# dluvizon/deephar

Measured on NVIDIA H100. Metric: frames/sec (256x256, 16-frame clips, b32), higher is better.
Workload: dtype bf16x3 split (fp32 accumulate, wgmma)

## Files before the change

deephar_b200/csrc/conv_sep.cu:

```cuda
#include "tc_common.cuh"

namespace tcs {
using namespace tc;
using R = tc::Roles<2, 1>;
constexpr int WARP_EPI0 = R::WARP_EPI0, WARP_TMA = R::WARP_TMA, WARP_PATCH = R::WARP_PATCH, NTHREADS = R::NTHREADS,
              REGS_PROD = R::REGS_PROD, REGS_EPI = R::REGS_EPI, REGS_CTRL = R::REGS_CTRL;

constexpr int A_BYTES = BM * 64;
constexpr int NWG = 128;
constexpr int NPW = 1;
constexpr int NA = 4;
constexpr int NB = 3;
constexpr int NP = 3;

struct SepParams {
    TcParams t;
    int patch_stride;
    int patch_bytes;
    int ry, fn;
    int dbg;
};

template <int KS, int TW, bool SHARE, bool BNPRO, bool LO>
__global__ void __launch_bounds__(NTHREADS, 1)
sep_tma_kernel(const __grid_constant__ SepParams SP, const __grid_constant__ CUtensorMap map_hi,
               const __grid_constant__ CUtensorMap map_lo, const __grid_constant__ CUtensorMap map_x) {
    constexpr int PAD = KS / 2;
    constexpr int PC = TW + 2 * PAD;
    constexpr int NR = 4 + KS - 1;
#ifdef DH_ABLATE
    const int DBG = SP.dbg;
#else
    constexpr int DBG = 0;
#endif
    const TcParams& P = SP.t;
    extern __shared__ __align__(1024) uint8_t smem_raw[];
    if (smem_u32(smem_raw) & 1023u) __trap();
    uint8_t* smem = smem_raw;
    const int tid = threadIdx.x;
    const int warp = tid >> 5, lane = tid & 31;
    constexpr bool want_lo = LO;
    const int b_bytes = P.bn_cta * 64;
    uint8_t* b_ring = smem + NA * 2 * A_BYTES;
    uint8_t* patch0 = b_ring + NB * 2 * b_bytes;
    uint64_t* bars = reinterpret_cast<uint64_t*>(patch0 + NP * SP.patch_stride);
    constexpr int NB_A = NA + 2 * NA;
    const uint32_t bar_full0 = smem_u32(bars), bar_empty0 = smem_u32(bars + NA), bar_fullb0 = smem_u32(bars + NB_A),
                   bar_emptyb0 = smem_u32(bars + NB_A + NB), bar_pfull0 = smem_u32(bars + NB_A + 2 * NB),
                   bar_pempty0 = smem_u32(bars + NB_A + 2 * NB + NP);
    const int n0 = blockIdx.y * P.bn_cta;
    const int nkb = P.n_kblocks;
    const uint32_t my_rank = SHARE ? cluster_ctarank() : 0u;

    if (warp == WARP_TMA && lane == 0) {
        tma_prefetch_desc(&map_hi);
        if (want_lo) tma_prefetch_desc(&map_lo);
        tma_prefetch_desc(&map_x);
        for (int s = 0; s < NA; ++s) {
            mbar_init(bar_full0 + 8 * s, SHARE ? 1u : (uint32_t)NWG);
            mbar_init(bar_empty0 + 16 * s, (SHARE ? 2u : 1u) * R::EPQ);
            mbar_init(bar_empty0 + 16 * s + 8, (SHARE ? 2u : 1u) * R::EPQ);
        }
        for (int s = 0; s < NB; ++s) {
            mbar_init(bar_fullb0 + 8 * s, 1);
            mbar_init(bar_emptyb0 + 8 * s, R::EPQ);
        }
        for (int s = 0; s < NP; ++s) {
            mbar_init(bar_pfull0 + 8 * s, 1);
            mbar_init(bar_pempty0 + 8 * s, NWG);
        }
        fence_barrier_init();
    }
    if (SHARE) cluster_sync_all(); else __syncthreads();

    const int tiles_mine = ((int)P.n_mtiles - (int)blockIdx.x + (int)gridDim.x - 1) / (int)gridDim.x;
    const int total_g = tiles_mine * nkb;
    const int n_own = SHARE ? (total_g - (int)my_rank + 1) / 2 : total_g;

    if (warp < WARP_EPI0) {
        reg_prod<REGS_PROD, R::LAUNCH_REGS>();
        const ConvParams& c = P.c;
        const int w = warp >> 2;
        const int tw = tid & (NWG - 1);
        const int cp = tw & 15;
        const int blk = tw >> 4;
        constexpr int XB = TW / 4;
        const int strip = blk / XB, xb = blk - strip * XB;
        const int fn = (strip * 4) / SP.ry, ry = (strip * 4) - fn * SP.ry;
        const int prr = SP.ry + 2 * PAD;
        const float* pbase0 = reinterpret_cast<const float*>(patch0) +
                             ((size_t)((fn * prr + ry) * PC + xb * 4)) * SBK + cp * 2;
        const int row0 = strip * 4 * TW + xb * 4;
        const float lowb = c.pre_relu ? 0.f : -3.402823466e38f;
        unsigned colmask = 0;
        if (BNPRO) {
#pragma unroll
            for (int q = 0; q < NR; ++q) {
                const int ix = xb * 4 + q - PAD;
                if (ix >= 0 && ix < TW) colmask |= 1u << q;
            }
        }
        float2 wt[KS][KS];
        auto load_taps = [&](int jn) {
            const int gn = SHARE ? 2 * jn + (int)my_rank : jn;
            const int kbn = gn % nkb;
            const float* wp = c.w_dw + kbn * SBK + cp * 2;
#pragma unroll
            for (int a = 0; a < KS; ++a)
#pragma unroll
                for (int b = 0; b < KS; ++b)
                    wt[a][b] = __ldg(reinterpret_cast<const float2*>(wp + (size_t)(a * KS + b) * c.Cin));
        };
        if (w < n_own) load_taps(w);
        for (int j = w; j < n_own; j += NPW) {
            const int pb_i = j % NP;
            const uint32_t pfull = bar_pfull0 + 8 * pb_i, pempty = bar_pempty0 + 8 * pb_i;
            const float* pbase = pbase0 + (size_t)pb_i * (SP.patch_stride / 4);
            const int g = SHARE ? 2 * j + (int)my_rank : j;
            const int ti = g / nkb, kb = g - ti * nkb;
            const int ch = kb * SBK + cp * 2;
            float2 acc[4][4];
#pragma unroll
            for (int o = 0; o < 4; ++o)
#pragma unroll
                for (int q = 0; q < 4; ++q) acc[o][q] = make_float2(0.f, 0.f);
            float2 ps = make_float2(1.f, 1.f), pb = make_float2(0.f, 0.f);
            unsigned rowmask = 0;
            if (BNPRO) {
                ps = __ldg(reinterpret_cast<const float2*>(c.pre_scale + ch));
                pb = __ldg(reinterpret_cast<const float2*>(c.pre_shift + ch));
                const int t = blockIdx.x + ti * gridDim.x;
                const int y0 = SP.fn > 1 ? 0 : ((t * BM) / TW) % c.H;
#pragma unroll
                for (int r = 0; r < NR; ++r) {
                    const int iy = y0 + ry + r - PAD;
                    if (iy >= 0 && iy < c.H) rowmask |= 1u << r;
                }
            }

            if (!(DBG & 2)) mbar_wait_relaxed(pfull, (uint32_t)((j / NP) & 1), (DBG & 2048) ? 32u : 0u);
            auto load_row = [&](int r, float2* in) {
#pragma unroll
                for (int q = 0; q < NR; ++q) {
                    float2 v = *reinterpret_cast<const float2*>(pbase + (r * PC + q) * SBK);
                    if (BNPRO) v = ffma2(v, ps, pb);
                    v = make_float2(fmaxf(v.x, lowb), fmaxf(v.y, lowb));
                    if (BNPRO && !(((rowmask >> r) & 1u) && ((colmask >> q) & 1u))) v = make_float2(0.f, 0.f);
                    in[q] = v;
                }
            };
            if (!(DBG & 1)) {
                float2 inb[2][NR];
                load_row(0, inb[0]);
#pragma unroll
                for (int r = 0; r < NR; ++r) {
                    if (r + 1 < NR) load_row(r + 1, inb[(r + 1) & 1]);
                    const float2* in = inb[r & 1];
#pragma unroll
                    for (int kx = 0; kx < KS; ++kx)
#pragma unroll
                        for (int o = 0; o < 4; ++o) {
                            const int ky = r - o;
                            if (ky >= 0 && ky < KS) {
#pragma unroll
                                for (int q = 0; q < 4; ++q) acc[o][q] = ffma2(wt[ky][kx], in[q + kx], acc[o][q]);
                            }
                        }
                }
            }
            if (j + NPW < n_own) load_taps(j + NPW);
            if (!(DBG & 2)) mbar_arrive(pempty);

            const int s = g % NA;
            const uint32_t it = (uint32_t)(g / NA);
            wait_stage_free(bar_empty0, s, it, (DBG & 2048) ? 32u : 0u);
            uint8_t* a_hi = smem + (size_t)s * (2 * A_BYTES);
            uint8_t* a_lo = a_hi + A_BYTES;
#pragma unroll
            for (int o = 0; o < 4; ++o)
#pragma unroll
                for (int q = 0; q < 4; ++q) {
                    uint32_t hi, lo;
                    split2(acc[o][q].x, acc[o][q].y, hi, lo);
                    const uint32_t off = swz64(row0 + o * TW + q, cp * 2);
                    *reinterpret_cast<uint32_t*>(a_hi + off) = hi;
                    if (want_lo) *reinterpret_cast<uint32_t*>(a_lo + off) = lo;
                }
            fence_proxy_async();
            if (SHARE) {
                asm volatile("bar.sync %0, %1;" ::"r"(1 + w), "r"(NWG) : "memory");
                if (tw == 0) {
                    mbar_arrive(bar_full0 + 8 * s);
                    const uint32_t peer = my_rank ^ 1u;
                    const uint32_t peer_full = mapa_peer(bar_full0 + 8 * s, peer);
                    if (!(DBG & 8)) {
                        bulk_s2peer(mapa_peer(smem_u32(a_hi), peer), smem_u32(a_hi), A_BYTES, peer_full);
                        if (want_lo) bulk_s2peer(mapa_peer(smem_u32(a_lo), peer), smem_u32(a_lo), A_BYTES, peer_full);
                    }
                }
            } else {
                mbar_arrive(bar_full0 + 8 * s);
            }
        }
    } else if (warp < WARP_TMA) {
        reg_inc<REGS_EPI>();
        const int wg = (warp - WARP_EPI0) >> 2, wt = tid - 32 * WARP_EPI0 - 128 * wg;
        float acc[R::MH][ACC_N];
        const uint64_t dbase = make_desc64(smem_u32(smem) + (uint32_t)(wg * 64 * 64));
        const uint64_t dbase_b = make_desc64(smem_u32(b_ring));
        const uint32_t sta16 = (2 * A_BYTES) >> 4, stb16 = (uint32_t)(2 * b_bytes) >> 4, alo16 = A_BYTES >> 4,
                       blo16 = (uint32_t)b_bytes >> 4;
        for (int ti = 0; ti < tiles_mine; ++ti) {
            const int g0 = ti * nkb;
            wg_tile<R::MH, SBK / 16, LO>(
                P.bn_cta, acc, nkb, 0u, alo16, blo16, !(DBG & 64),
                [&](int kb, uint64_t& da, uint64_t& db) {
                    const int g = g0 + kb, s = g % NA, sb = g % NB;
                    if (!(DBG & 128)) mbar_wait(bar_full0 + 8 * s, (uint32_t)(g / NA) & 1);
                    mbar_wait(bar_fullb0 + 8 * sb, (uint32_t)(g / NB) & 1);
                    da = dbase + (uint64_t)((uint32_t)s * sta16);
                    db = dbase_b + (uint64_t)((uint32_t)sb * stb16);
                },
                [&](int kb) {
                    const int g = g0 + kb, s = g % NA;
                    wg_release<SHARE>(bar_empty0 + 16 * s + 8 * ((g / NA) & 1), wg, wt, my_rank ^ 1u);
                    if (wt == 0) mbar_arrive(bar_emptyb0 + 8 * (g % NB));
                });
            wg_epilogue<R::MH>(P, acc, ((int)blockIdx.x + ti * (int)gridDim.x) * BM + 64 * wg, n0, wt);
        }
    } else {
        reg_dec<REGS_CTRL>();
        if (warp == WARP_TMA) {
            if (lane == 0) {
                const uint32_t tx = (DBG & 16) ? 0u : (uint32_t)(want_lo ? 2 : 1) * (uint32_t)b_bytes;
                const uint32_t tx_a = (DBG & 8) ? 0u : (uint32_t)(want_lo ? 2 : 1) * (uint32_t)A_BYTES;
                for (int g = 0; g < total_g; ++g) {
                    const int ti = g / nkb, kb = g - ti * nkb;
                    const int sb = g % NB;
                    const uint32_t itb = (uint32_t)(g / NB);
                    if (itb >= 1) mbar_wait_relaxed(bar_emptyb0 + 8 * sb, (itb - 1) & 1, (DBG & 2048) ? 64u : 0u);
                    const uint32_t full = bar_fullb0 + 8 * sb;
                    mbar_arrive_expect_tx(full, tx);
                    const uint32_t b_hi = smem_u32(b_ring + (size_t)sb * (2 * b_bytes));
                    const uint32_t b_lo = b_hi + (uint32_t)b_bytes;
                    if (!(DBG & 16)) {
                        tma_load_2d(b_hi, &map_hi, kb * SBK, n0, full);
                        if (want_lo) tma_load_2d(b_lo, &map_lo, kb * SBK, n0, full);
                    }
                    if (SHARE && (uint32_t)(g & 1) != my_rank) {
                        const int sa = g % NA;
                        wait_stage_free(bar_empty0, sa, (uint32_t)(g / NA));
                        mbar_arrive_expect_tx(bar_full0 + 8 * sa, tx_a);
                    }
                }
            }
        } else if (warp == WARP_PATCH) {
            if (lane == 0 && !(DBG & 2)) {
                const ConvParams& c = P.c;
                auto coords = [&](int j, int& kb, int& nf, int& y0) {
                    const int g = SHARE ? 2 * j + (int)my_rank : j;
                    const int ti = g / nkb;
                    kb = g - ti * nkb;
                    const int t = blockIdx.x + ti * gridDim.x;
                    const int grow = (t * BM) / TW;
                    nf = grow / c.H;
                    y0 = grow - nf * c.H;
                };
                for (int j = 0; j < n_own; ++j) {
                    int kb, nf, y0;
                    coords(j, kb, nf, y0);
                    const int w = j % NP;
                    const int pfd = (DBG & 1024) ? 2 : (DBG & 4096) ? 4 : (DBG & 8192) ? 9 : 0;
                    if (pfd && j + pfd < n_own) {
                        int kb2, nf2, y2;
                        coords(j + pfd, kb2, nf2, y2);
                        tma_prefetch_4d(&map_x, kb2 * SBK, -PAD, y2 - PAD, nf2);
                    }
                    mbar_wait_relaxed(bar_pempty0 + 8 * w, (uint32_t)(((j / NP) & 1) ^ 1), (DBG & 2048) ? 64u : 0u);
                    const uint32_t pf = bar_pfull0 + 8 * w;
                    mbar_arrive_expect_tx(pf, (uint32_t)SP.patch_bytes);
                    tma_load_4d(smem_u32(patch0 + (size_t)w * SP.patch_stride), &map_x, kb * SBK, -PAD, y0 - PAD, nf, pf);
                }
            }
        }
    }
    if (SHARE) cluster_sync_all(); else __syncthreads();
}

static bool make_map_x(CUtensorMap* map, const ConvParams& p, int pc, int prr, int fn) {
    EncodeTiledFn enc = get_encode();
    if (!enc) return false;
    cuuint64_t dims[4] = {(cuuint64_t)p.Cin, (cuuint64_t)p.W, (cuuint64_t)p.H, (cuuint64_t)p.N};
    cuuint64_t strides[3] = {(cuuint64_t)p.ldx * 4, (cuuint64_t)p.W * p.ldx * 4, (cuuint64_t)p.H * p.W * p.ldx * 4};
    cuuint32_t box[4] = {(cuuint32_t)SBK, (cuuint32_t)pc, (cuuint32_t)prr, (cuuint32_t)fn};
    cuuint32_t estr[4] = {1, 1, 1, 1};
    return enc(map, CU_TENSOR_MAP_DATA_TYPE_FLOAT32, 4, const_cast<float*>(p.x), dims, strides, box, estr,
               CU_TENSOR_MAP_INTERLEAVE_NONE, CU_TENSOR_MAP_SWIZZLE_NONE, CU_TENSOR_MAP_L2_PROMOTION_L2_256B,
               CU_TENSOR_MAP_FLOAT_OOB_FILL_NONE) == CUDA_SUCCESS;
}

}

bool dh_sep_tma_supported(const dh_ctx* ctx, const ConvParams& p, const dh_packed_w* packed) {
    if (!ctx->sep_tma) return false;
    if (!packed || !packed->hi || !packed->lo) return false;
    if (!(p.kh == p.kw && (p.kh == 3 || p.kh == 5)) || p.sh != 1 || p.sw != 1) return false;
    if (p.Ho != p.H || p.Wo != p.W) return false;
    if (p.pre_scale && ((reinterpret_cast<uintptr_t>(p.pre_scale) & 7) || (reinterpret_cast<uintptr_t>(p.pre_shift) & 7))) return false;
    if (!(p.W == 32 || p.W == 16 || p.W == 8)) return false;
    const int tr = tc::BM / p.W;
    if (tr <= p.H ? (p.H % tr) != 0 : (tr % p.H) != 0) return false;
    if ((p.Cin % tcs::SBK) != 0 || (p.ldx & 3)) return false;
    if ((reinterpret_cast<uintptr_t>(p.x) & 15) || (reinterpret_cast<uintptr_t>(p.w_dw) & 7)) return false;
    if (packed->cout_pad != dh_tc_cout_pad(p.Cout) || packed->k < p.Cin) return false;
    return true;
}

int dh_launch_sep_tma(dh_ctx* ctx, const ConvParams& p, const dh_packed_w* packed, int precision, cudaStream_t s) {
    using namespace tc;
    using namespace tcs;
    SepParams SP;
    TcParams& P = SP.t;
    P.c = p;
    P.c.K = p.Cin;
    P.k_pad = packed->k;
    P.n_kblocks = p.Cin / SBK;
    int gy;
    tile_n(p.Cout, &P.bn_cta, &gy);
    P.precision = (precision == 1) ? 1 : 3;
    P.ks = p.kh;
    P.n_mtiles = (p.M + BM - 1) / BM;
    P.stages = 2;
    const int pad = p.kh / 2;
    const int tr = BM / p.W;
    SP.ry = tr <= p.H ? tr : p.H;
    SP.fn = tr <= p.H ? 1 : tr / p.H;
    const int pc = p.W + 2 * pad, prr = SP.ry + 2 * pad;
    SP.patch_bytes = SBK * 4 * pc * prr * SP.fn;
    SP.patch_stride = (SP.patch_bytes + 1023) / 1024 * 1024;
#ifdef DH_ABLATE
    SP.dbg = ctx->dbg;
    P.dbg = ctx->dbg;
#else
    SP.dbg = 0;
    P.dbg = 0;
#endif
    const size_t smem = (size_t)NA * 2 * A_BYTES + (size_t)NB * 2 * P.bn_cta * 64 + NP * (size_t)SP.patch_stride + 512;
    if (smem > 227 * 1024) {
        dh_set_error("dh_launch_sep_tma: tile does not fit shared memory");
        return -1;
    }
    CUtensorMap map_hi, map_lo, map_x;
    if (!make_map_b64(&map_hi, packed->hi, packed->k, packed->cout_pad, P.bn_cta) ||
        !make_map_b64(&map_lo, packed->lo, packed->k, packed->cout_pad, P.bn_cta) ||
        !make_map_x(&map_x, p, pc, prr, SP.fn)) {
        dh_set_error("dh_launch_sep_tma: cuTensorMapEncodeTiled failed");
        return -1;
    }
    int gx = ctx->num_sms / gy;
    if (gx < 1) gx = 1;
    if (gx > P.n_mtiles) gx = P.n_mtiles;
    dim3 grid(gx, gy);
    const bool share = gy % 2 == 0 && ctx->share_a;
    cudaError_t e = cudaSuccess;
#define DH_SEP_LAUNCH_(KS_, TW_, BN_, LO_)                                                                              \
    do {                                                                                                         \
        if (share) {                                                                                             \
            e = ensure_smem<sep_tma_kernel<KS_, TW_, true, BN_, LO_>>(smem); \
            if (e == cudaSuccess) {                                                                              \
                cudaLaunchConfig_t cfg = {};                                                                     \
                cfg.gridDim = grid; cfg.blockDim = dim3(NTHREADS); cfg.dynamicSmemBytes = smem; cfg.stream = s;  \
                cudaLaunchAttribute at[1];                                                                       \
                at[0].id = cudaLaunchAttributeClusterDimension;                                                  \
                at[0].val.clusterDim.x = 1; at[0].val.clusterDim.y = 2; at[0].val.clusterDim.z = 1;              \
                cfg.attrs = at; cfg.numAttrs = 1;                                                                \
                e = cudaLaunchKernelEx(&cfg, sep_tma_kernel<KS_, TW_, true, BN_, LO_>, SP, map_hi, map_lo, map_x);    \
            }                                                                                                    \
        } else {                                                                                                 \
            e = ensure_smem<sep_tma_kernel<KS_, TW_, false, BN_, LO_>>(smem); \
            if (e == cudaSuccess) sep_tma_kernel<KS_, TW_, false, BN_, LO_><<<grid, NTHREADS, smem, s>>>(SP, map_hi, map_lo, map_x); \
        }                                                                                                        \
    } while (0)
#define DH_SEP_LAUNCH_P(KS_, TW_, BN_) do { if (P.precision == 3) DH_SEP_LAUNCH_(KS_, TW_, BN_, true); else DH_SEP_LAUNCH_(KS_, TW_, BN_, false); } while (0)
#define DH_SEP_LAUNCH(KS_, TW_) do { if (p.pre_scale) DH_SEP_LAUNCH_P(KS_, TW_, true); else DH_SEP_LAUNCH_P(KS_, TW_, false); } while (0)
    if (p.kh == 5) {
        if (p.W == 32) DH_SEP_LAUNCH(5, 32); else if (p.W == 16) DH_SEP_LAUNCH(5, 16); else DH_SEP_LAUNCH(5, 8);
    } else {
        if (p.W == 32) DH_SEP_LAUNCH(3, 32); else if (p.W == 16) DH_SEP_LAUNCH(3, 16); else DH_SEP_LAUNCH(3, 8);
    }
#undef DH_SEP_LAUNCH
#undef DH_SEP_LAUNCH_P
#undef DH_SEP_LAUNCH_
    if (e != cudaSuccess) {
        dh_set_error("dh_launch_sep_tma: launch setup failed: %s", cudaGetErrorString(e));
        return (int)e;
    }
    return 0;
}
```

deephar_b200/csrc/tc_common.cuh:

```cuda
#pragma once
#include <cuda.h>
#include <cuda_bf16.h>
#include "common.cuh"
#include "conv_params.cuh"

namespace tc {


constexpr int BM = 128;
constexpr int BK = 64;
constexpr int NPROD = 256;
constexpr int MAX_BN_CTA = 96;
constexpr int ACC_N = MAX_BN_CTA / 2;
template <int Q, int NPW = 2>
struct Roles {
    static constexpr int EPQ = Q;
    static constexpr int MH = 2 / Q;
    static constexpr int NEPI = 128 * Q;
    static constexpr int WARP_EPI0 = 4 * NPW;
    static constexpr int WARP_TMA = WARP_EPI0 + 4 * Q, WARP_PATCH = WARP_TMA + 2;
    static constexpr int NTHREADS = 32 * (WARP_TMA + 4);
    static constexpr int REGS_PROD = Q == 1 ? 168 : (NPW == 1 ? 192 : 80), REGS_EPI = 144, REGS_CTRL = 32;
    static constexpr int LAUNCH_REGS = NTHREADS <= 512 ? 128 : 96;
    static_assert(128 * NPW * REGS_PROD + NEPI * REGS_EPI + 128 * REGS_CTRL <= NTHREADS * LAUNCH_REGS,
                  "setmaxnreg budget exceeds the CTA's register allocation: the last setmaxnreg.inc would never return");
};
constexpr int A_TILE_BYTES = BM * 128;
constexpr int MAX_STAGES = 4;

struct TcParams {
    ConvParams c;
    int n_kblocks;
    int bn_cta;
    int stages;
    int precision;
    int ks;
    int k_pad;
    int n_mtiles;
    int dbg;
};

__device__ __forceinline__ uint32_t smem_u32(const void* p) { return (uint32_t)__cvta_generic_to_shared(p); }

__device__ __forceinline__ void mbar_init(uint32_t bar, uint32_t count) {
    asm volatile("mbarrier.init.shared::cta.b64 [%0], %1;" ::"r"(bar), "r"(count));
}
__device__ __forceinline__ void mbar_arrive(uint32_t bar) {
    asm volatile("{\n .reg .b64 st;\n mbarrier.arrive.shared::cta.b64 st, [%0];\n}" ::"r"(bar) : "memory");
}
__device__ __forceinline__ void mbar_arrive_expect_tx(uint32_t bar, uint32_t bytes) {
    asm volatile("{\n .reg .b64 st;\n mbarrier.arrive.expect_tx.shared::cta.b64 st, [%0], %1;\n}" ::"r"(bar), "r"(bytes)
                 : "memory");
}
__device__ __forceinline__ void mbar_wait(uint32_t bar, uint32_t parity) {
    uint32_t ok;
    do {
        asm volatile(
            "{\n .reg .pred p;\n mbarrier.try_wait.parity.shared::cta.b64 p, [%1], %2;\n selp.u32 %0, 1, 0, p;\n}"
            : "=r"(ok)
            : "r"(bar), "r"(parity)
            : "memory");
    } while (!ok);
}
__device__ __forceinline__ void mbar_wait_relaxed(uint32_t bar, uint32_t parity, uint32_t ns) {
    uint32_t ok;
    for (;;) {
        asm volatile(
            "{\n .reg .pred p;\n mbarrier.try_wait.parity.shared::cta.b64 p, [%1], %2;\n selp.u32 %0, 1, 0, p;\n}"
            : "=r"(ok)
            : "r"(bar), "r"(parity)
            : "memory");
        if (ok) break;
        if (ns) __nanosleep(ns);
    }
}
__device__ __forceinline__ void fence_barrier_init() { asm volatile("fence.mbarrier_init.release.cluster;" ::: "memory"); }
__device__ __forceinline__ void fence_proxy_async() { asm volatile("fence.proxy.async.shared::cta;" ::: "memory"); }

__device__ __forceinline__ void tma_load_2d(uint32_t dst, const CUtensorMap* map, int c0, int c1, uint32_t bar) {
    asm volatile(
        "cp.async.bulk.tensor.2d.shared::cluster.global.mbarrier::complete_tx::bytes [%0], [%1, {%2, %3}], [%4];"
        ::"r"(dst), "l"(map), "r"(c0), "r"(c1), "r"(bar)
        : "memory");
}
__device__ __forceinline__ void tma_prefetch_desc(const CUtensorMap* map) {
    asm volatile("prefetch.tensormap [%0];" ::"l"(map) : "memory");
}
__device__ __forceinline__ uint32_t cluster_ctarank() {
    uint32_t r;
    asm volatile("mov.u32 %0, %%cluster_ctarank;" : "=r"(r));
    return r;
}
__device__ __forceinline__ uint32_t mapa_peer(uint32_t local_addr, uint32_t peer) {
    uint32_t r;
    asm volatile("mapa.shared::cluster.u32 %0, %1, %2;" : "=r"(r) : "r"(local_addr), "r"(peer));
    return r;
}
__device__ __forceinline__ void cluster_sync_all() {
    asm volatile("barrier.cluster.arrive.release.aligned;\n\tbarrier.cluster.wait.acquire.aligned;" ::: "memory");
}
__device__ __forceinline__ void bulk_s2peer(uint32_t dst_cluster, uint32_t src_cta, uint32_t bytes, uint32_t bar_cluster) {
    asm volatile("cp.async.bulk.shared::cluster.shared::cta.mbarrier::complete_tx::bytes [%0], [%1], %2, [%3];"
                 ::"r"(dst_cluster), "r"(src_cta), "r"(bytes), "r"(bar_cluster)
                 : "memory");
}
template <int R> __device__ __forceinline__ void reg_inc() { asm volatile("setmaxnreg.inc.sync.aligned.u32 %0;" ::"n"(R)); }
template <int R> __device__ __forceinline__ void reg_dec() { asm volatile("setmaxnreg.dec.sync.aligned.u32 %0;" ::"n"(R)); }
template <int R, int LAUNCH> __device__ __forceinline__ void reg_prod() {
    if constexpr (R > LAUNCH) reg_inc<R>();
    else if constexpr (R < LAUNCH) reg_dec<R>();
}
__device__ __forceinline__ void mbar_arrive_cluster(uint32_t bar_cluster) {
    asm volatile("mbarrier.arrive.release.cluster.shared::cluster.b64 _, [%0];" ::"r"(bar_cluster) : "memory");
}

__device__ __forceinline__ void wgmma_fence() { asm volatile("wgmma.fence.sync.aligned;" ::: "memory"); }
__device__ __forceinline__ void wgmma_commit() { asm volatile("wgmma.commit_group.sync.aligned;" ::: "memory"); }
template <int N> __device__ __forceinline__ void wgmma_wait() { asm volatile("wgmma.wait_group.sync.aligned %0;" ::"n"(N) : "memory"); }
__device__ __forceinline__ void acc_fence(float& r) { asm volatile("" : "+f"(r)::"memory"); }
template <int N> __device__ __forceinline__ void wgmma_bf16(float* d, uint64_t a, uint64_t b, uint32_t acc);
template <> __device__ __forceinline__ void wgmma_bf16<16>(float* d, uint64_t a, uint64_t b, uint32_t acc) {
    asm volatile(
        "{\n .reg .pred p;\n setp.ne.b32 p, %10, 0;\n"
        " wgmma.mma_async.sync.aligned.m64n16k16.f32.bf16.bf16 {%0, %1, %2, %3, %4, %5, %6, %7}, %8, %9, p, 1, 1, 0, 0;\n}"
        : "+f"(d[0]), "+f"(d[1]), "+f"(d[2]), "+f"(d[3]), "+f"(d[4]), "+f"(d[5]), "+f"(d[6]), "+f"(d[7])
        : "l"(a), "l"(b), "r"(acc));
}
template <> __device__ __forceinline__ void wgmma_bf16<32>(float* d, uint64_t a, uint64_t b, uint32_t acc) {
    asm volatile(
        "{\n .reg .pred p;\n setp.ne.b32 p, %18, 0;\n"
        " wgmma.mma_async.sync.aligned.m64n32k16.f32.bf16.bf16 {%0, %1, %2, %3, %4, %5, %6, %7, %8, %9, %10, %11, %12, %13, %14, %15}, %16, %17, p, 1, 1, 0, 0;\n}"
        : "+f"(d[0]), "+f"(d[1]), "+f"(d[2]), "+f"(d[3]), "+f"(d[4]), "+f"(d[5]), "+f"(d[6]), "+f"(d[7]), "+f"(d[8]), "+f"(d[9]), "+f"(d[10]), "+f"(d[11]), "+f"(d[12]), "+f"(d[13]), "+f"(d[14]), "+f"(d[15])
        : "l"(a), "l"(b), "r"(acc));
}
template <> __device__ __forceinline__ void wgmma_bf16<48>(float* d, uint64_t a, uint64_t b, uint32_t acc) {
    asm volatile(
        "{\n .reg .pred p;\n setp.ne.b32 p, %26, 0;\n"
        " wgmma.mma_async.sync.aligned.m64n48k16.f32.bf16.bf16 {%0, %1, %2, %3, %4, %5, %6, %7, %8, %9, %10, %11, %12, %13, %14, %15, %16, %17, %18, %19, %20, %21, %22, %23}, %24, %25, p, 1, 1, 0, 0;\n}"
        : "+f"(d[0]), "+f"(d[1]), "+f"(d[2]), "+f"(d[3]), "+f"(d[4]), "+f"(d[5]), "+f"(d[6]), "+f"(d[7]), "+f"(d[8]), "+f"(d[9]), "+f"(d[10]), "+f"(d[11]), "+f"(d[12]), "+f"(d[13]), "+f"(d[14]), "+f"(d[15]), "+f"(d[16]), "+f"(d[17]), "+f"(d[18]), "+f"(d[19]), "+f"(d[20]), "+f"(d[21]), "+f"(d[22]), "+f"(d[23])
        : "l"(a), "l"(b), "r"(acc));
}
template <> __device__ __forceinline__ void wgmma_bf16<64>(float* d, uint64_t a, uint64_t b, uint32_t acc) {
    asm volatile(
        "{\n .reg .pred p;\n setp.ne.b32 p, %34, 0;\n"
        " wgmma.mma_async.sync.aligned.m64n64k16.f32.bf16.bf16 {%0, %1, %2, %3, %4, %5, %6, %7, %8, %9, %10, %11, %12, %13, %14, %15, %16, %17, %18, %19, %20, %21, %22, %23, %24, %25, %26, %27, %28, %29, %30, %31}, %32, %33, p, 1, 1, 0, 0;\n}"
        : "+f"(d[0]), "+f"(d[1]), "+f"(d[2]), "+f"(d[3]), "+f"(d[4]), "+f"(d[5]), "+f"(d[6]), "+f"(d[7]), "+f"(d[8]), "+f"(d[9]), "+f"(d[10]), "+f"(d[11]), "+f"(d[12]), "+f"(d[13]), "+f"(d[14]), "+f"(d[15]), "+f"(d[16]), "+f"(d[17]), "+f"(d[18]), "+f"(d[19]), "+f"(d[20]), "+f"(d[21]), "+f"(d[22]), "+f"(d[23]), "+f"(d[24]), "+f"(d[25]), "+f"(d[26]), "+f"(d[27]), "+f"(d[28]), "+f"(d[29]), "+f"(d[30]), "+f"(d[31])
        : "l"(a), "l"(b), "r"(acc));
}
template <> __device__ __forceinline__ void wgmma_bf16<80>(float* d, uint64_t a, uint64_t b, uint32_t acc) {
    asm volatile(
        "{\n .reg .pred p;\n setp.ne.b32 p, %42, 0;\n"
        " wgmma.mma_async.sync.aligned.m64n80k16.f32.bf16.bf16 {%0, %1, %2, %3, %4, %5, %6, %7, %8, %9, %10, %11, %12, %13, %14, %15, %16, %17, %18, %19, %20, %21, %22, %23, %24, %25, %26, %27, %28, %29, %30, %31, %32, %33, %34, %35, %36, %37, %38, %39}, %40, %41, p, 1, 1, 0, 0;\n}"
        : "+f"(d[0]), "+f"(d[1]), "+f"(d[2]), "+f"(d[3]), "+f"(d[4]), "+f"(d[5]), "+f"(d[6]), "+f"(d[7]), "+f"(d[8]), "+f"(d[9]), "+f"(d[10]), "+f"(d[11]), "+f"(d[12]), "+f"(d[13]), "+f"(d[14]), "+f"(d[15]), "+f"(d[16]), "+f"(d[17]), "+f"(d[18]), "+f"(d[19]), "+f"(d[20]), "+f"(d[21]), "+f"(d[22]), "+f"(d[23]), "+f"(d[24]), "+f"(d[25]), "+f"(d[26]), "+f"(d[27]), "+f"(d[28]), "+f"(d[29]), "+f"(d[30]), "+f"(d[31]), "+f"(d[32]), "+f"(d[33]), "+f"(d[34]), "+f"(d[35]), "+f"(d[36]), "+f"(d[37]), "+f"(d[38]), "+f"(d[39])
        : "l"(a), "l"(b), "r"(acc));
}
template <> __device__ __forceinline__ void wgmma_bf16<96>(float* d, uint64_t a, uint64_t b, uint32_t acc) {
    asm volatile(
        "{\n .reg .pred p;\n setp.ne.b32 p, %50, 0;\n"
        " wgmma.mma_async.sync.aligned.m64n96k16.f32.bf16.bf16 {%0, %1, %2, %3, %4, %5, %6, %7, %8, %9, %10, %11, %12, %13, %14, %15, %16, %17, %18, %19, %20, %21, %22, %23, %24, %25, %26, %27, %28, %29, %30, %31, %32, %33, %34, %35, %36, %37, %38, %39, %40, %41, %42, %43, %44, %45, %46, %47}, %48, %49, p, 1, 1, 0, 0;\n}"
        : "+f"(d[0]), "+f"(d[1]), "+f"(d[2]), "+f"(d[3]), "+f"(d[4]), "+f"(d[5]), "+f"(d[6]), "+f"(d[7]), "+f"(d[8]), "+f"(d[9]), "+f"(d[10]), "+f"(d[11]), "+f"(d[12]), "+f"(d[13]), "+f"(d[14]), "+f"(d[15]), "+f"(d[16]), "+f"(d[17]), "+f"(d[18]), "+f"(d[19]), "+f"(d[20]), "+f"(d[21]), "+f"(d[22]), "+f"(d[23]), "+f"(d[24]), "+f"(d[25]), "+f"(d[26]), "+f"(d[27]), "+f"(d[28]), "+f"(d[29]), "+f"(d[30]), "+f"(d[31]), "+f"(d[32]), "+f"(d[33]), "+f"(d[34]), "+f"(d[35]), "+f"(d[36]), "+f"(d[37]), "+f"(d[38]), "+f"(d[39]), "+f"(d[40]), "+f"(d[41]), "+f"(d[42]), "+f"(d[43]), "+f"(d[44]), "+f"(d[45]), "+f"(d[46]), "+f"(d[47])
        : "l"(a), "l"(b), "r"(acc));
}

__device__ __forceinline__ uint64_t make_desc(uint32_t smem_addr) {
    return (uint64_t)((smem_addr >> 4) & 0x3FFF) | (1ull << 16) | ((uint64_t)(1024 >> 4) << 32) | (1ull << 62);
}


__device__ __forceinline__ void split2(float a, float b, uint32_t& hi, uint32_t& lo) {
    __nv_bfloat162 h = __floats2bfloat162_rn(a, b);
    float ra = a - __low2float(h), rb = b - __high2float(h);
    __nv_bfloat162 l = __floats2bfloat162_rn(ra, rb);
    hi = *reinterpret_cast<uint32_t*>(&h);
    lo = *reinterpret_cast<uint32_t*>(&l);
}

__device__ __forceinline__ uint32_t swz(int row, int k) {
    return (uint32_t)(row * 128 + ((((k >> 3) ^ (row & 7)) << 4) | ((k & 7) << 1)));
}


constexpr int SBK = 32;
__device__ __forceinline__ void tma_load_4d(uint32_t dst, const CUtensorMap* map, int c0, int c1, int c2, int c3,
                                            uint32_t bar) {
    asm volatile(
        "cp.async.bulk.tensor.4d.shared::cluster.global.mbarrier::complete_tx::bytes [%0], [%1, {%2, %3, %4, %5}], [%6];"
        ::"r"(dst), "l"(map), "r"(c0), "r"(c1), "r"(c2), "r"(c3), "r"(bar)
        : "memory");
}

__device__ __forceinline__ void tma_prefetch_4d(const CUtensorMap* map, int c0, int c1, int c2, int c3) {
    asm volatile("cp.async.bulk.prefetch.tensor.4d.L2.global [%0, {%1, %2, %3, %4}];"
                 ::"l"(map), "r"(c0), "r"(c1), "r"(c2), "r"(c3) : "memory");
}

__device__ __forceinline__ uint64_t make_desc64(uint32_t smem_addr) {
    return (uint64_t)((smem_addr >> 4) & 0x3FFF) | (1ull << 16) | ((uint64_t)(512 >> 4) << 32) | (2ull << 62);
}
__device__ __forceinline__ uint32_t swz64(int row, int k) {
    return (uint32_t)(row * 64 + ((((k >> 3) ^ ((row >> 1) & 3)) << 4) | ((k & 7) << 1)));
}

__device__ __forceinline__ float4 lds128(uint32_t a) {
    float4 v;
    asm volatile("ld.shared.v4.f32 {%0, %1, %2, %3}, [%4];" : "=f"(v.x), "=f"(v.y), "=f"(v.z), "=f"(v.w) : "r"(a) : "memory");
    return v;
}

__device__ __forceinline__ void wait_stage_free(uint32_t bar_empty0, int s, uint32_t it, uint32_t ns = 0) {
    if (it >= 1) mbar_wait_relaxed(bar_empty0 + 16 * s + 8 * ((it - 1) & 1), ((it - 1) >> 1) & 1, ns);
}


template <int N, int MH>
__device__ __forceinline__ void acc_fence_all(float (&acc)[MH][ACC_N]) {
#pragma unroll
    for (int h = 0; h < MH; ++h)
#pragma unroll
        for (int i = 0; i < N / 2; ++i) acc_fence(acc[h][i]);
}

template <int N, int MH, int NK16, bool LO>
__device__ __forceinline__ void wg_issue_kblock(float (&acc)[MH][ACC_N], uint64_t da, uint32_t a_half16, uint32_t alo16,
                                                uint64_t db, uint32_t blo16, bool first) {
    wgmma_fence();
#pragma unroll
    for (int k = 0; k < NK16; ++k) {
        const uint32_t acc0 = (first && k == 0) ? 0u : 1u;
#pragma unroll
        for (int h = 0; h < MH; ++h) {
            const uint64_t a = da + (uint64_t)(h * a_half16 + 2 * k);
            wgmma_bf16<N>(acc[h], a, db + 2 * k, acc0);
            if (LO) {
                wgmma_bf16<N>(acc[h], a + alo16, db + 2 * k, 1u);
                wgmma_bf16<N>(acc[h], a, db + blo16 + 2 * k, 1u);
            }
        }
    }
    wgmma_commit();
}

template <int N, int MH, int NK16, bool LO, class Stage, class Release>
__device__ __forceinline__ void wg_tile_n(float (&acc)[MH][ACC_N], int nkb, uint32_t a_half16, uint32_t alo16,
                                          uint32_t blo16, bool mma, Stage& stage, Release& release) {
    for (int kb = 0; kb < nkb; ++kb) {
        uint64_t da, db;
        stage(kb, da, db);
        if (mma) {
            acc_fence_all<N>(acc);
            wg_issue_kblock<N, MH, NK16, LO>(acc, da, a_half16, alo16, db, blo16, kb == 0);
        }
        wgmma_wait<1>();
        acc_fence_all<N>(acc);
        if (kb > 0) release(kb - 1);
    }
    wgmma_wait<0>();
    acc_fence_all<N>(acc);
    release(nkb - 1);
}

template <int MH, int NK16, bool LO, class Stage, class Release>
__device__ __forceinline__ void wg_tile(int bn, float (&acc)[MH][ACC_N], int nkb, uint32_t a_half16, uint32_t alo16,
                                        uint32_t blo16, bool mma, Stage&& stage, Release&& release) {
    switch (bn) {
    case 16: wg_tile_n<16, MH, NK16, LO>(acc, nkb, a_half16, alo16, blo16, mma, stage, release); break;
    case 32: wg_tile_n<32, MH, NK16, LO>(acc, nkb, a_half16, alo16, blo16, mma, stage, release); break;
    case 48: wg_tile_n<48, MH, NK16, LO>(acc, nkb, a_half16, alo16, blo16, mma, stage, release); break;
    case 64: wg_tile_n<64, MH, NK16, LO>(acc, nkb, a_half16, alo16, blo16, mma, stage, release); break;
    case 80: wg_tile_n<80, MH, NK16, LO>(acc, nkb, a_half16, alo16, blo16, mma, stage, release); break;
    default: wg_tile_n<96, MH, NK16, LO>(acc, nkb, a_half16, alo16, blo16, mma, stage, release); break;
    }
}

template <bool SHARE>
__device__ __forceinline__ void wg_release(uint32_t bar, int wg, int wt, uint32_t peer) {
    asm volatile("bar.sync %0, 128;" ::"r"(4 + wg) : "memory");
    if (wt == 0) {
        mbar_arrive(bar);
        if (SHARE) mbar_arrive_cluster(mapa_peer(bar, peer));
    }
}

__device__ __forceinline__ size_t res1_src(const ConvParams& c, int m) {
    if (!c.up1) return (size_t)m;
    const int hw = c.Ho * c.Wo;
    const int n = m / hw, rem = m - n * hw;
    const int y = rem / c.Wo, x = rem - y * c.Wo;
    return ((size_t)n * (c.Ho >> 1) + (y >> 1)) * (size_t)(c.Wo >> 1) + (size_t)(x >> 1);
}

__device__ __forceinline__ float2 ldg2(const float* p) { return __ldg(reinterpret_cast<const float2*>(p)); }

template <int MH>
__device__ __forceinline__ void wg_epilogue(const TcParams& P, const float (&acc)[MH][ACC_N], int m0, int n0, int wt) {
    const ConvParams& c = P.c;
#ifdef DH_ABLATE
    if (P.dbg & 32) return;
#endif
    const int rq = 16 * (wt >> 5) + ((wt & 31) >> 2);
    const int cq = 2 * (wt & 3);
    const bool v2 = !((c.ldo | c.Cout) & 1) && !(reinterpret_cast<uintptr_t>(c.out) & 7) &&
                    (!c.res0 || (!(c.ldr0 & 1) && !(reinterpret_cast<uintptr_t>(c.res0) & 7))) &&
                    (!c.res1 || (!(c.ldr1 & 1) && !(reinterpret_cast<uintptr_t>(c.res1) & 7))) &&
                    (!c.post_scale || (!(reinterpret_cast<uintptr_t>(c.post_scale) & 7) &&
                                       !(reinterpret_cast<uintptr_t>(c.post_shift) & 7)));
    const bool relu = c.post_relu != 0, has_post = c.post_scale != nullptr;
    constexpr int JC = 6;
    static_assert((ACC_N / 4) % JC == 0, "column groups per batch");
#pragma unroll
    for (int h = 0; h < MH; ++h)
#pragma unroll
        for (int hr = 0; hr < 2; ++hr) {
            const int m = m0 + 64 * h + rq + 8 * hr;
            if (m >= c.M) continue;
            float* orow = c.out + (size_t)m * c.ldo;
            const float* r0row = c.res0 ? c.res0 + (size_t)m * c.ldr0 : nullptr;
            const float* r1row = c.res1 ? c.res1 + res1_src(c, m) * c.ldr1 : nullptr;
            if (MH == 1 && v2) {
#pragma unroll
                for (int j0 = 0; j0 < ACC_N / 4; j0 += JC) {
                    if (8 * j0 >= P.bn_cta) break;
                    float2 sc[JC], sh[JC], ra[JC], rb[JC];
#pragma unroll
                    for (int jj = 0; jj < JC; ++jj) {
                        const int co = n0 + 8 * (j0 + jj) + cq;
                        if (8 * (j0 + jj) < P.bn_cta && co < c.Cout) {
                            if (has_post) { sc[jj] = ldg2(c.post_scale + co); sh[jj] = ldg2(c.post_shift + co); }
                            if (r0row) ra[jj] = ldg2(r0row + co);
                            if (r1row) rb[jj] = ldg2(r1row + co);
                        }
                    }
#pragma unroll
                    for (int jj = 0; jj < JC; ++jj) {
                        const int j = j0 + jj;
                        const int co = n0 + 8 * j + cq;
                        if (8 * j < P.bn_cta && co < c.Cout) {
                            float2 v = make_float2(acc[h][4 * j + 2 * hr], acc[h][4 * j + 2 * hr + 1]);
                            if (has_post) v = ffma2(v, sc[jj], sh[jj]);
                            if (relu) v = make_float2(fmaxf(v.x, 0.f), fmaxf(v.y, 0.f));
                            if (r0row) v = fadd2(v, ra[jj]);
                            if (r1row) v = fadd2(v, rb[jj]);
                            *reinterpret_cast<float2*>(orow + co) = v;
                        }
                    }
                }
                continue;
            }
#pragma unroll
            for (int j = 0; j < ACC_N / 4; ++j) {
                if (8 * j >= P.bn_cta) break;
                const int co = n0 + 8 * j + cq;
                float2 v = make_float2(acc[h][4 * j + 2 * hr], acc[h][4 * j + 2 * hr + 1]);
                if (v2) {
                    if (co < c.Cout) {
                        if (has_post) v = ffma2(v, ldg2(c.post_scale + co), ldg2(c.post_shift + co));
                        if (relu) v = make_float2(fmaxf(v.x, 0.f), fmaxf(v.y, 0.f));
                        if (r0row) v = fadd2(v, ldg2(r0row + co));
                        if (r1row) v = fadd2(v, ldg2(r1row + co));
                        *reinterpret_cast<float2*>(orow + co) = v;
                    }
                } else {
#pragma unroll
                    for (int e = 0; e < 2; ++e) {
                        const int cc = co + e;
                        if (cc < c.Cout) {
                            float t = e ? v.y : v.x;
                            if (has_post) t = fmaf(t, __ldg(c.post_scale + cc), __ldg(c.post_shift + cc));
                            if (relu) t = fmaxf(t, 0.f);
                            if (r0row) t += __ldg(r0row + cc);
                            if (r1row) t += __ldg(r1row + cc);
                            orow[cc] = t;
                        }
                    }
                }
            }
        }
}

typedef CUresult (*EncodeTiledFn)(CUtensorMap*, CUtensorMapDataType, cuuint32_t, void*, const cuuint64_t*,
                                  const cuuint64_t*, const cuuint32_t*, const cuuint32_t*, CUtensorMapInterleave,
                                  CUtensorMapSwizzle, CUtensorMapL2promotion, CUtensorMapFloatOOBfill);

static inline EncodeTiledFn get_encode() {
    static EncodeTiledFn fn = nullptr;
    if (!fn) {
        void* p = nullptr;
        cudaDriverEntryPointQueryResult qres;
        if (cudaGetDriverEntryPoint("cuTensorMapEncodeTiled", &p, cudaEnableDefault, &qres) == cudaSuccess &&
            qres == cudaDriverEntryPointSuccess)
            fn = (EncodeTiledFn)p;
    }
    return fn;
}

static inline bool make_map(CUtensorMap* map, const void* base, int k_pad, int rows, int box_rows) {
    EncodeTiledFn enc = get_encode();
    if (!enc) return false;
    cuuint64_t dims[2] = {(cuuint64_t)k_pad, (cuuint64_t)rows};
    cuuint64_t strides[1] = {(cuuint64_t)k_pad * 2};
    cuuint32_t box[2] = {(cuuint32_t)BK, (cuuint32_t)box_rows};
    cuuint32_t estr[2] = {1, 1};
    CUresult r = enc(map, CU_TENSOR_MAP_DATA_TYPE_BFLOAT16, 2, const_cast<void*>(base), dims, strides, box, estr,
                     CU_TENSOR_MAP_INTERLEAVE_NONE, CU_TENSOR_MAP_SWIZZLE_128B, CU_TENSOR_MAP_L2_PROMOTION_L2_256B,
                     CU_TENSOR_MAP_FLOAT_OOB_FILL_NONE);
    return r == CUDA_SUCCESS;
}

static inline bool make_map_b64(CUtensorMap* map, const void* base, int k_pad, int rows, int box_rows) {
    EncodeTiledFn enc = get_encode();
    if (!enc) return false;
    cuuint64_t dims[2] = {(cuuint64_t)k_pad, (cuuint64_t)rows};
    cuuint64_t strides[1] = {(cuuint64_t)k_pad * 2};
    cuuint32_t box[2] = {(cuuint32_t)SBK, (cuuint32_t)box_rows};
    cuuint32_t estr[2] = {1, 1};
    return enc(map, CU_TENSOR_MAP_DATA_TYPE_BFLOAT16, 2, const_cast<void*>(base), dims, strides, box, estr,
               CU_TENSOR_MAP_INTERLEAVE_NONE, CU_TENSOR_MAP_SWIZZLE_64B, CU_TENSOR_MAP_L2_PROMOTION_L2_256B,
               CU_TENSOR_MAP_FLOAT_OOB_FILL_NONE) == CUDA_SUCCESS;
}


template <auto Kernel>
static inline cudaError_t ensure_smem(size_t smem) {
    static size_t cur = 0;
    if (smem <= cur) return cudaSuccess;
    cudaError_t e = cudaFuncSetAttribute(Kernel, cudaFuncAttributeMaxDynamicSharedMemorySize, (int)smem);
    if (e == cudaSuccess) cur = smem;
    return e;
}


static inline void tile_n(int cout, int* bn_cta, int* gy) {
    const int cp = (cout + 15) / 16 * 16;
    const int g = (cp + MAX_BN_CTA - 1) / MAX_BN_CTA;
    *bn_cta = ((cp + g - 1) / g + 15) / 16 * 16;
    *gy = g;
}

}
```

Before: 2652.

## Stage separable-conv epilogue through shared memory with TMA stores and residual loads

```diff
diff --git a/deephar_b200/csrc/conv_sep.cu b/deephar_b200/csrc/conv_sep.cu
--- a/deephar_b200/csrc/conv_sep.cu
+++ b/deephar_b200/csrc/conv_sep.cu
@@ -11,20 +11,69 @@
 constexpr int NPW = 1;
 constexpr int NA = 4;
 constexpr int NB = 3;
-constexpr int NP = 3;
+constexpr int NP_MAX = 3;
+constexpr int STAGE_BOX = BM * 64;
+constexpr int STAGE_HALF = STAGE_BOX / 2;
 
 struct SepParams {
     TcParams t;
     int patch_stride;
     int patch_bytes;
+    int np;
+    int stage_off;
+    int bar_off;
     int ry, fn;
     int dbg;
 };
 
+__device__ __forceinline__ void sep_epilogue_staged(const TcParams& P, const float (&acc)[1][ACC_N], int m0, int n0,
+                                                    int wt, uint32_t half, uint32_t bnv, bool res1) {
+    const ConvParams& c = P.c;
+    const int rq = 16 * (wt >> 5) + ((wt & 31) >> 2);
+    const int cq = 2 * (wt & 3);
+    const bool relu = c.post_relu != 0, has_post = c.post_scale != nullptr, res0 = c.res0 != nullptr;
+    constexpr int JC = 6;
+    static_assert((ACC_N / 4) % JC == 0, "column groups per batch");
+#pragma unroll
+    for (int hr = 0; hr < 2; ++hr) {
+        const int r = rq + 8 * hr;
+        const int m = m0 + r;
+        if (m >= c.M) continue;
+        const float* r1row = res1 ? c.res1 + res1_src(c, m) * c.ldr1 : nullptr;
+        const uint32_t srow = half + r * 64;
+        const int sw = (r >> 1) & 3;
+#pragma unroll
+        for (int j0 = 0; j0 < ACC_N / 4; j0 += JC) {
+            if (8 * j0 >= P.bn_cta) break;
+            float2 rb[JC];
+#pragma unroll
+            for (int jj = 0; jj < JC; ++jj) {
+                const int co = n0 + 8 * (j0 + jj) + cq;
+                if (r1row && 8 * (j0 + jj) < P.bn_cta && co < c.Cout) rb[jj] = ldg2(r1row + co);
+            }
+#pragma unroll
+            for (int jj = 0; jj < JC; ++jj) {
+                const int j = j0 + jj;
+                const int col = 8 * j + cq;
+                if (8 * j < P.bn_cta && n0 + col < c.Cout) {
+                    const uint32_t sp = srow + (j >> 1) * STAGE_BOX + ((((j & 1) * 2 + (cq >> 2)) ^ sw) << 4) + (cq & 3) * 4;
+                    float2 v = make_float2(acc[0][4 * j + 2 * hr], acc[0][4 * j + 2 * hr + 1]);
+                    if (has_post) v = ffma2(v, lds64(bnv + 4 * col), lds64(bnv + 4 * (MAX_BN_CTA + col)));
+                    if (relu) v = make_float2(fmaxf(v.x, 0.f), fmaxf(v.y, 0.f));
+                    if (res0) v = fadd2(v, lds64(sp));
+                    if (r1row) v = fadd2(v, rb[jj]);
+                    sts64(sp, v);
+                }
+            }
+        }
+    }
+}
+
 template <int KS, int TW, bool SHARE, bool BNPRO, bool LO>
 __global__ void __launch_bounds__(NTHREADS, 1)
 sep_tma_kernel(const __grid_constant__ SepParams SP, const __grid_constant__ CUtensorMap map_hi,
-               const __grid_constant__ CUtensorMap map_lo, const __grid_constant__ CUtensorMap map_x) {
+               const __grid_constant__ CUtensorMap map_lo, const __grid_constant__ CUtensorMap map_x,
+               const __grid_constant__ CUtensorMap map_o, const __grid_constant__ CUtensorMap map_r) {
     constexpr int PAD = KS / 2;
     constexpr int PC = TW + 2 * PAD;
     constexpr int NR = 4 + KS - 1;
@@ -41,13 +90,19 @@
     const int warp = tid >> 5, lane = tid & 31;
     constexpr bool want_lo = LO;
     const int b_bytes = P.bn_cta * 64;
+    const int NP = SP.np;
+    const bool staged = SP.stage_off != 0;
     uint8_t* b_ring = smem + NA * 2 * A_BYTES;
     uint8_t* patch0 = b_ring + NB * 2 * b_bytes;
-    uint64_t* bars = reinterpret_cast<uint64_t*>(patch0 + NP * SP.patch_stride);
+    uint8_t* stage = smem + SP.stage_off;
+    float* bnv = reinterpret_cast<float*>(stage + BM * P.bn_cta * 4);
+    uint64_t* bars = reinterpret_cast<uint64_t*>(smem + SP.bar_off);
     constexpr int NB_A = NA + 2 * NA;
     const uint32_t bar_full0 = smem_u32(bars), bar_empty0 = smem_u32(bars + NA), bar_fullb0 = smem_u32(bars + NB_A),
                    bar_emptyb0 = smem_u32(bars + NB_A + NB), bar_pfull0 = smem_u32(bars + NB_A + 2 * NB),
-                   bar_pempty0 = smem_u32(bars + NB_A + 2 * NB + NP);
+                   bar_pempty0 = smem_u32(bars + NB_A + 2 * NB + NP_MAX),
+                   bar_sready0 = smem_u32(bars + NB_A + 2 * NB + 2 * NP_MAX),
+                   bar_ofull0 = smem_u32(bars + NB_A + 2 * NB + 2 * NP_MAX + 2);
     const int n0 = blockIdx.y * P.bn_cta;
     const int nkb = P.n_kblocks;
     const uint32_t my_rank = SHARE ? cluster_ctarank() : 0u;
@@ -68,6 +123,14 @@
         for (int s = 0; s < NP; ++s) {
             mbar_init(bar_pfull0 + 8 * s, 1);
             mbar_init(bar_pempty0 + 8 * s, NWG);
+        }
+        if (staged) {
+            tma_prefetch_desc(&map_o);
+            if (P.c.res0) tma_prefetch_desc(&map_r);
+            for (int h = 0; h < 2; ++h) {
+                mbar_init(bar_sready0 + 8 * h, 1);
+                mbar_init(bar_ofull0 + 8 * h, 128);
+            }
         }
         fence_barrier_init();
     }
@@ -112,8 +175,8 @@
                     wt[a][b] = __ldg(reinterpret_cast<const float2*>(wp + (size_t)(a * KS + b) * c.Cin));
         };
         if (w < n_own) load_taps(w);
-        for (int j = w; j < n_own; j += NPW) {
-            const int pb_i = j % NP;
+        static_assert(NPW == 1, "the carried patch index steps one K-block per iteration");
+        for (int j = w, pb_i = 0, pu = 0; j < n_own; ++j, pb_i = (pb_i + 1 == NP) ? 0 : pb_i + 1, pu ^= (pb_i == 0)) {
             const uint32_t pfull = bar_pfull0 + 8 * pb_i, pempty = bar_pempty0 + 8 * pb_i;
             const float* pbase = pbase0 + (size_t)pb_i * (SP.patch_stride / 4);
             const int g = SHARE ? 2 * j + (int)my_rank : j;
@@ -138,7 +201,7 @@
                 }
             }
 
-            if (!(DBG & 2)) mbar_wait_relaxed(pfull, (uint32_t)((j / NP) & 1), (DBG & 2048) ? 32u : 0u);
+            if (!(DBG & 2)) mbar_wait_relaxed(pfull, (uint32_t)pu, (DBG & 2048) ? 32u : 0u);
             auto load_row = [&](int r, float2* in) {
 #pragma unroll
                 for (int q = 0; q < NR; ++q) {
@@ -210,8 +273,15 @@
         const uint64_t dbase_b = make_desc64(smem_u32(b_ring));
         const uint32_t sta16 = (2 * A_BYTES) >> 4, stb16 = (uint32_t)(2 * b_bytes) >> 4, alo16 = A_BYTES >> 4,
                        blo16 = (uint32_t)b_bytes >> 4;
-        for (int ti = 0; ti < tiles_mine; ++ti) {
-            const int g0 = ti * nkb;
+        if (staged && P.c.post_scale) {
+            const int i = tid - 32 * WARP_EPI0, col = i % P.bn_cta, co = n0 + col;
+            if (i < 2 * P.bn_cta)
+                bnv[(i < P.bn_cta ? 0 : MAX_BN_CTA) + col] =
+                    co < P.c.Cout ? __ldg((i < P.bn_cta ? P.c.post_scale : P.c.post_shift) + co) : 0.f;
+            asm volatile("bar.sync 6, %0;" ::"n"(128 * R::EPQ) : "memory");
+        }
+        uint32_t ph = 0;
+        for (int t = cta_x(), g0 = 0; t < (int)P.n_mtiles; t += gridDim.x, g0 += nkb, ph ^= 1u) {
             wg_tile<R::MH, SBK / 16, LO>(
                 P.bn_cta, acc, nkb, 0u, alo16, blo16, !(DBG & 64),
                 [&](int kb, uint64_t& da, uint64_t& db) {
@@ -226,7 +296,16 @@
                     wg_release<SHARE>(bar_empty0 + 16 * s + 8 * ((g / NA) & 1), wg, wt, my_rank ^ 1u);
                     if (wt == 0) mbar_arrive(bar_emptyb0 + 8 * (g % NB));
                 });
-            wg_epilogue<R::MH>(P, acc, ((int)blockIdx.x + ti * (int)gridDim.x) * BM + 64 * wg, n0, wt);
+            const int m0 = t * BM + 64 * wg;
+            if (staged) {
+                mbar_wait(bar_sready0 + 8 * wg, ph);
+                sep_epilogue_staged(P, acc, m0, n0, wt, smem_u32(stage) + wg * STAGE_HALF, smem_u32(bnv),
+                                    P.c.res1 && !(DBG & 32));
+                fence_proxy_async();
+                mbar_arrive(bar_ofull0 + 8 * wg);
+            } else {
+                wg_epilogue<R::MH>(P, acc, m0, n0, wt);
+            }
         }
     } else {
         reg_dec<REGS_CTRL>();
@@ -254,6 +333,43 @@
                     }
                 }
             }
+        } else if (warp == WARP_TMA + 1) {
+            if (staged && lane == 0) {
+                const ConvParams& c = P.c;
+                const int nbox = (min(P.bn_cta, c.Cout - n0) + 15) / 16;
+                const bool gio = !(DBG & 32), res = c.res0 && gio;
+                const uint32_t st0 = smem_u32(stage);
+                uint32_t ph = 0;
+                for (int t = cta_x() - (int)gridDim.x; t < (int)P.n_mtiles; t += gridDim.x) {
+#pragma unroll 1
+                    for (int h = 0; h < 2; ++h) {
+                        const uint32_t sh = st0 + h * STAGE_HALF;
+                        if (t >= 0) {
+                            const int mh = t * BM + 64 * h;
+                            mbar_wait(bar_ofull0 + 8 * h, ph);
+                            if (gio && mh < c.M) {
+#pragma unroll 1
+                                for (int b = 0; b < nbox; ++b) tma_store_2d(&map_o, n0 + 16 * b, mh, sh + b * STAGE_BOX);
+                                bulk_commit();
+                            }
+                            bulk_wait_read<0>();
+                        }
+                        const int mn = (t + (int)gridDim.x) * BM + 64 * h;
+                        if (t + (int)gridDim.x < (int)P.n_mtiles) {
+                            const uint32_t bar = bar_sready0 + 8 * h;
+                            if (res && mn < c.M) {
+                                mbar_arrive_expect_tx(bar, (uint32_t)(nbox * STAGE_HALF));
+#pragma unroll 1
+                                for (int b = 0; b < nbox; ++b) tma_load_2d(sh + b * STAGE_BOX, &map_r, n0 + 16 * b, mn, bar);
+                            } else {
+                                mbar_arrive(bar);
+                            }
+                        }
+                    }
+                    if (t >= 0) ph ^= 1u;
+                }
+                bulk_wait<0>();
+            }
         } else if (warp == WARP_PATCH) {
             if (lane == 0 && !(DBG & 2)) {
                 const ConvParams& c = P.c;
@@ -266,17 +382,16 @@
                     nf = grow / c.H;
                     y0 = grow - nf * c.H;
                 };
-                for (int j = 0; j < n_own; ++j) {
+                for (int j = 0, w = 0, u = 0; j < n_own; ++j, w = (w + 1 == NP) ? 0 : w + 1, u ^= (w == 0)) {
                     int kb, nf, y0;
                     coords(j, kb, nf, y0);
-                    const int w = j % NP;
                     const int pfd = (DBG & 1024) ? 2 : (DBG & 4096) ? 4 : (DBG & 8192) ? 9 : 0;
                     if (pfd && j + pfd < n_own) {
                         int kb2, nf2, y2;
                         coords(j + pfd, kb2, nf2, y2);
                         tma_prefetch_4d(&map_x, kb2 * SBK, -PAD, y2 - PAD, nf2);
                     }
-                    mbar_wait_relaxed(bar_pempty0 + 8 * w, (uint32_t)(((j / NP) & 1) ^ 1), (DBG & 2048) ? 64u : 0u);
+                    mbar_wait_relaxed(bar_pempty0 + 8 * w, (uint32_t)(u ^ 1), (DBG & 2048) ? 64u : 0u);
                     const uint32_t pf = bar_pfull0 + 8 * w;
                     mbar_arrive_expect_tx(pf, (uint32_t)SP.patch_bytes);
                     tma_load_4d(smem_u32(patch0 + (size_t)w * SP.patch_stride), &map_x, kb * SBK, -PAD, y0 - PAD, nf, pf);
@@ -345,15 +460,27 @@
     SP.dbg = 0;
     P.dbg = 0;
 #endif
-    const size_t smem = (size_t)NA * 2 * A_BYTES + (size_t)NB * 2 * P.bn_cta * 64 + NP * (size_t)SP.patch_stride + 512;
-    if (smem > 227 * 1024) {
+    auto al = [](const void* q, uintptr_t a) { return (reinterpret_cast<uintptr_t>(q) & (a - 1)) == 0; };
+    const bool staged = al(p.out, 16) && !(p.ldo & 3) && !(p.Cout & 1) &&
+                        (!p.res0 || (al(p.res0, 16) && !(p.ldr0 & 3))) && (!p.res1 || (al(p.res1, 8) && !(p.ldr1 & 1)));
+    const size_t fixed = (size_t)NA * 2 * A_BYTES + (size_t)NB * 2 * P.bn_cta * 64;
+    const size_t stage_bytes = staged ? (size_t)BM * P.bn_cta * 4 + 2 * MAX_BN_CTA * 4 : 0;
+    const size_t budget = 227 * 1024, bar_bytes = 512;
+    const size_t np = fixed + stage_bytes + bar_bytes < budget ? (budget - fixed - stage_bytes - bar_bytes) / SP.patch_stride : 0;
+    SP.np = np < (size_t)NP_MAX ? (int)np : NP_MAX;
+    SP.stage_off = staged ? (int)(fixed + (size_t)SP.np * SP.patch_stride) : 0;
+    SP.bar_off = (int)(fixed + (size_t)SP.np * SP.patch_stride + stage_bytes);
+    const size_t smem = (size_t)SP.bar_off + bar_bytes;
+    if (SP.np < 1 || smem > 227 * 1024) {
         dh_set_error("dh_launch_sep_tma: tile does not fit shared memory");
         return -1;
     }
-    CUtensorMap map_hi, map_lo, map_x;
+    CUtensorMap map_hi, map_lo, map_x, map_o = {}, map_r = {};
     if (!make_map_b64(&map_hi, packed->hi, packed->k, packed->cout_pad, P.bn_cta) ||
         !make_map_b64(&map_lo, packed->lo, packed->k, packed->cout_pad, P.bn_cta) ||
-        !make_map_x(&map_x, p, pc, prr, SP.fn)) {
+        !make_map_x(&map_x, p, pc, prr, SP.fn) ||
+        (staged && !make_map_f32_c16(&map_o, p.out, p.Cout, p.M, p.ldo, BM / 2)) ||
+        (staged && p.res0 && !make_map_f32_c16(&map_r, p.res0, p.Cout, p.M, p.ldr0, BM / 2))) {
         dh_set_error("dh_launch_sep_tma: cuTensorMapEncodeTiled failed");
         return -1;
     }
@@ -374,11 +501,12 @@
                 at[0].id = cudaLaunchAttributeClusterDimension;                                                  \
                 at[0].val.clusterDim.x = 1; at[0].val.clusterDim.y = 2; at[0].val.clusterDim.z = 1;              \
                 cfg.attrs = at; cfg.numAttrs = 1;                                                                \
-                e = cudaLaunchKernelEx(&cfg, sep_tma_kernel<KS_, TW_, true, BN_, LO_>, SP, map_hi, map_lo, map_x);    \
+                e = cudaLaunchKernelEx(&cfg, sep_tma_kernel<KS_, TW_, true, BN_, LO_>, SP, map_hi, map_lo, map_x, \
+                                       map_o, map_r);                                                            \
             }                                                                                                    \
         } else {                                                                                                 \
             e = ensure_smem<sep_tma_kernel<KS_, TW_, false, BN_, LO_>>(smem); \
-            if (e == cudaSuccess) sep_tma_kernel<KS_, TW_, false, BN_, LO_><<<grid, NTHREADS, smem, s>>>(SP, map_hi, map_lo, map_x); \
+            if (e == cudaSuccess) sep_tma_kernel<KS_, TW_, false, BN_, LO_><<<grid, NTHREADS, smem, s>>>(SP, map_hi, map_lo, map_x, map_o, map_r); \
         }                                                                                                        \
     } while (0)
 #define DH_SEP_LAUNCH_P(KS_, TW_, BN_) do { if (P.precision == 3) DH_SEP_LAUNCH_(KS_, TW_, BN_, true); else DH_SEP_LAUNCH_(KS_, TW_, BN_, false); } while (0)
diff --git a/deephar_b200/csrc/tc_common.cuh b/deephar_b200/csrc/tc_common.cuh
--- a/deephar_b200/csrc/tc_common.cuh
+++ b/deephar_b200/csrc/tc_common.cuh
@@ -41,6 +41,11 @@
 };
 
 __device__ __forceinline__ uint32_t smem_u32(const void* p) { return (uint32_t)__cvta_generic_to_shared(p); }
+__device__ __forceinline__ int cta_x() {
+    int r;
+    asm volatile("mov.u32 %0, %%ctaid.x;" : "=r"(r));
+    return r;
+}
 
 __device__ __forceinline__ void mbar_init(uint32_t bar, uint32_t count) {
     asm volatile("mbarrier.init.shared::cta.b64 [%0], %1;" ::"r"(bar), "r"(count));
@@ -194,6 +199,16 @@
                  ::"l"(map), "r"(c0), "r"(c1), "r"(c2), "r"(c3) : "memory");
 }
 
+__device__ __forceinline__ void tma_store_2d(const CUtensorMap* map, int c0, int c1, uint32_t src) {
+    asm volatile("cp.async.bulk.tensor.2d.global.shared::cta.bulk_group [%0, {%1, %2}], [%3];"
+                 ::"l"(map), "r"(c0), "r"(c1), "r"(src) : "memory");
+}
+__device__ __forceinline__ void bulk_commit() { asm volatile("cp.async.bulk.commit_group;" ::: "memory"); }
+template <int N> __device__ __forceinline__ void bulk_wait_read() {
+    asm volatile("cp.async.bulk.wait_group.read %0;" ::"n"(N) : "memory");
+}
+template <int N> __device__ __forceinline__ void bulk_wait() { asm volatile("cp.async.bulk.wait_group %0;" ::"n"(N) : "memory"); }
+
 __device__ __forceinline__ uint64_t make_desc64(uint32_t smem_addr) {
     return (uint64_t)((smem_addr >> 4) & 0x3FFF) | (1ull << 16) | ((uint64_t)(512 >> 4) << 32) | (2ull << 62);
 }
@@ -205,6 +220,14 @@
     float4 v;
     asm volatile("ld.shared.v4.f32 {%0, %1, %2, %3}, [%4];" : "=f"(v.x), "=f"(v.y), "=f"(v.z), "=f"(v.w) : "r"(a) : "memory");
     return v;
+}
+__device__ __forceinline__ float2 lds64(uint32_t a) {
+    float2 v;
+    asm volatile("ld.shared.v2.f32 {%0, %1}, [%2];" : "=f"(v.x), "=f"(v.y) : "r"(a) : "memory");
+    return v;
+}
+__device__ __forceinline__ void sts64(uint32_t a, float2 v) {
+    asm volatile("st.shared.v2.f32 [%0], {%1, %2};" ::"r"(a), "f"(v.x), "f"(v.y) : "memory");
 }
 
 __device__ __forceinline__ void wait_stage_free(uint32_t bar_empty0, int s, uint32_t it, uint32_t ns = 0) {
@@ -418,6 +441,18 @@
                CU_TENSOR_MAP_FLOAT_OOB_FILL_NONE) == CUDA_SUCCESS;
 }
 
+static inline bool make_map_f32_c16(CUtensorMap* map, const float* base, int cols, int rows, int ld, int box_rows) {
+    EncodeTiledFn enc = get_encode();
+    if (!enc) return false;
+    cuuint64_t dims[2] = {(cuuint64_t)cols, (cuuint64_t)rows};
+    cuuint64_t strides[1] = {(cuuint64_t)ld * 4};
+    cuuint32_t box[2] = {16, (cuuint32_t)box_rows};
+    cuuint32_t estr[2] = {1, 1};
+    return enc(map, CU_TENSOR_MAP_DATA_TYPE_FLOAT32, 2, const_cast<float*>(base), dims, strides, box, estr,
+               CU_TENSOR_MAP_INTERLEAVE_NONE, CU_TENSOR_MAP_SWIZZLE_64B, CU_TENSOR_MAP_L2_PROMOTION_L2_256B,
+               CU_TENSOR_MAP_FLOAT_OOB_FILL_NONE) == CUDA_SUCCESS;
+}
+
 
 template <auto Kernel>
 static inline cudaError_t ensure_smem(size_t smem) {
```

Result: faster. 2701 (median of 6 runs) (+1.9%).
